# rvaser/rala

Measured on AMD Instinct MI355X. Metric: overlaps/sec (pile build + transitive reduction), higher is better.
Workload: dtype u16/u32 (+f64 compares)

## Files before the change

rala_amd/csrc/context.h:

```cpp
#pragma once

#include <hip/hip_runtime.h>
#include <stdint.h>

#include <algorithm>

#include <memory>
#include <string>
#include <vector>

#include "geom.h"
#include "host_pool.h"
#include "kernels.h"
#include "rala_hip.h"

namespace rala_hip {

struct HostOvl {
    uint32_t src;
    uint32_t a, b;
    Coords c;
    uint8_t strand;
    uint8_t dead;
    uint8_t type;
// ... 141 lines not shown
    uint32_t n_compute_units = 256;
    hipStream_t stream = nullptr;
    hipStream_t side = nullptr;
    hipStream_t aux = nullptr;
    bool use_side_stream = true;
    std::string err;
    hipEvent_t ev[12] = {};
    hipStream_t copy = nullptr;
    hipEvent_t ev_up[4] = {};
    bool upload_pending = false, upload_queued = false;
    const uint32_t* up_src[7] = {};
    const uint8_t* up_strand = nullptr;

    int64_t pool_per_read_x1000 = 1000;
    int64_t max_lds_read_len = 22000;
    int64_t debug_pile_stop_after = 99;
    int64_t host_threads = 0;
    std::unique_ptr<rala_hip::HostPool> pool;
    bool use_run_kernel = true;
    bool debug_fail_construct = false;
    uint32_t debug_pile_variant = 0;
    uint32_t debug_dedupe_list_cap = 0;
    uint32_t debug_fp_lds_limit = 0xFFFFFFFFu;
    uint32_t debug_fp_give_up = 0;
    int64_t debug_chunk_fail = -1;
    uint32_t debug_part_shift = 0;
    uint32_t debug_count_window = 0;
    bool use_bound_records = true;
    bool use_round_batches = true;
    rala_hip::DevBuf<uint32_t> d_round_log;

    uint64_t n_reads = 0;
    uint32_t max_read_len = 0;
    uint32_t n_class[rala_hip::kPileClasses] = {};
    rala_hip::DevBuf<uint32_t> d_class_order;
    rala_hip::DevBuf<uint32_t> d_seg_base;
    rala_hip::DevBuf<uint32_t> d_dense;
    std::vector<uint32_t> h_read_len;
    std::vector<uint64_t> h_pile_off;
    uint64_t pile_elems = 0;
    rala_hip::DevBuf<uint32_t> d_read_len;
    rala_hip::DevBuf<uint64_t> d_pile_off;
    rala_hip::DevBuf<uint16_t> d_pile;
    rala_hip::DevBuf<uint32_t> d_order, d_overflow;
    rala_hip::DevBuf<uint32_t> d_big_list[2], d_big_space;
    int64_t debug_big_caps = 0;
// ... 159 lines not shown
```

rala_amd/csrc/kernels.h:

```cpp
#pragma once

#include <hip/hip_runtime.h>
#include <stdint.h>

namespace rala_hip {

constexpr uint32_t kPadL = 848;

enum : uint32_t {
    kErrRegionCapacity = 1u,
    kErrPoolCapacity = 2u,
    kErrRawCapacity = 4u,
};

struct Interval {
    uint32_t first, second;
    uint32_t aux;
};

struct PileArgs {
    const uint32_t* read_len;
    const uint64_t* pile_off;
    uint16_t* pile;
    const uint32_t* ev_off;
// ... 214 lines not shown
void launch_sens_filter(const TailList& L, const uint32_t* begin, const uint32_t* end, const uint32_t* n_rep,
                        const uint32_t* rep_slot, const Interval* rep_pool, hipStream_t s);
void launch_finalize_states(const TailList& L, const uint8_t* alive, hipStream_t s);
void launch_list_targets(const uint32_t* off, uint32_t n, uint32_t* list, uint32_t* count, hipStream_t s);
void launch_list_members(const uint32_t* alive_reads, const uint8_t* touched, uint32_t n_alive, uint32_t world, uint32_t rank,
                         uint32_t* list, uint32_t* count, hipStream_t s);
struct SensSplitArgs {
    const uint32_t* read_len;
    const uint32_t* ev_off;
    const uint32_t* ev_cnt;
    uint32_t ev_stride;
    uint32_t ev_shift;
    const uint32_t* sens_off;
    const uint32_t* begin;
    const uint32_t* end;
    uint32_t* out[5];
    uint32_t* counts;
};
void launch_sens_split(const uint32_t* list, uint32_t bound, const uint32_t* n_dev, const SensSplitArgs& args, hipStream_t s);
void launch_status_clear(uint32_t* status, uint32_t bits, uint32_t* zero, hipStream_t s);
void launch_scatter_component_medians(const uint32_t* alive_reads, const uint8_t* touched, const uint16_t* cmed, uint32_t n_alive,
                                      uint16_t* out, hipStream_t s);
void launch_break_hills(const TailReads& R, uint32_t n_reads, hipStream_t s);
void launch_break_pits(const TailReads& R, const uint32_t* alive_reads, const uint8_t* touched, const uint16_t* comp_median,
                       uint32_t n_alive, hipStream_t s, const uint32_t* gate = nullptr);
void launch_retrim(const TailList& L, const TailReads& R, uint32_t promote, uint32_t round, uint32_t* dropped,
                   hipStream_t s, const uint32_t* gate = nullptr);
void launch_cc_edges(const TailList& L, const uint32_t* rank, uint32_t* edges, uint8_t* touched, uint32_t* label, uint32_t n_labels,
                     hipStream_t s);
void launch_refresh_types(const TailList& L, const TailReads& R, hipStream_t s);
hipError_t launch_tail_contain(const TailList& L, const TailReads& R, uint8_t* alive, uint32_t* const lists[6], uint32_t* zeroed21, uint32_t* const work[4],
                               uint32_t* base2, uint8_t* mark2, uint32_t* map, uint32_t* pack, uint32_t n_reads, uint32_t lds_limit, uint32_t debug_give_up, hipStream_t s);
void launch_count_zero_u8(const uint8_t* x, uint32_t n, uint32_t* out, hipStream_t s);
void launch_tail_init(const TailList& L, uint32_t n0, const TailReads& R, uint32_t* n_pits0, uint32_t n_reads, uint32_t* base2,
                      uint8_t* mark2, uint32_t* map, uint32_t* zero22, hipStream_t s);
struct ScanSpace;
bool launch_rank_pass(const uint8_t* alive, uint32_t* rank, uint32_t* alive_reads, uint32_t n_reads, ScanSpace& space, hipStream_t s);
bool launch_node_pass(const uint8_t* alive, uint32_t* node_rank, uint32_t* node_read, uint32_t* n_final, uint32_t n_reads,
                      ScanSpace& space, hipStream_t s);
bool launch_segment_pass(const TailList& L, const TailReads& R, uint32_t want_state, uint32_t want_round, uint32_t* base,
                         uint32_t* next, uint32_t* kept_item, const uint32_t* node_rank, uint32_t* e_src, uint32_t* e_dst,
                         uint32_t* e_len, ScanSpace& space, hipStream_t s);
bool launch_offsets_pass(const uint32_t* in, uint32_t* out, uint32_t* copy, uint32_t n, ScanSpace& space, hipStream_t s);
bool launch_pair_offsets_pass(const uint32_t* in0, const uint32_t* in1, uint32_t* out0, uint32_t* out1, uint32_t* totals, uint32_t n,
                              ScanSpace& space, hipStream_t s);

struct FixedPointList {
    const uint32_t *key, *target, *keeper;
    const uint32_t* count;
    uint32_t lds_limit = 0xFFFFFFFFu;
    uint32_t debug_give_up = 0;
};
size_t fixed_point_pack_words();
hipError_t launch_fixed_point_finish(const FixedPointList& list, uint32_t* base, uint32_t* map, uint32_t* pack, uint32_t* const work[4],
                                     uint32_t* sync8, uint32_t* error, uint32_t* rounds_out, hipStream_t s);
// ... 97 lines not shown
void launch_gzip_resolve(uint16_t* sym, const uint64_t* text_off, uint32_t n_true, uint64_t text_n, uint8_t* text, uint32_t* seg_crc,
                         uint32_t* flags, hipStream_t s);
uint32_t gzip_segment_bytes();
uint32_t gzip_crc_of_segments(const uint32_t* seg_crc, uint64_t text_n);

size_t scan_workspace_bytes(uint64_t n);
void launch_exclusive_scan(const uint32_t* in, uint32_t* out, uint64_t n, void* workspace, hipStream_t s);

void launch_tr_mark(const uint32_t* row_ptr, const uint32_t* adj_edge, const uint32_t* edge_src,
                    const uint32_t* edge_dst, const uint32_t* edge_len, uint32_t n_nodes, uint32_t first_edge,
                    uint32_t last_edge, uint8_t* marks, hipStream_t s);
void launch_tr_degree(const uint32_t* src, const uint32_t* dst, uint32_t n_nodes, uint32_t n_edges, uint32_t* deg,
                      uint32_t* bad, hipStream_t s);
void launch_tr_fill(const uint32_t* src, const uint32_t* dst, uint32_t n_nodes, uint32_t n_edges, uint32_t* cursor, uint32_t* adj,
                    hipStream_t s);
void launch_cc_init(uint32_t* label, uint32_t n, hipStream_t s);
void launch_cc_hook(const uint32_t* edges, uint32_t n_edges, uint32_t sample, uint32_t* label, uint32_t* changed,
                    hipStream_t s);
void launch_cc_compress(uint32_t* label, uint32_t n, hipStream_t s);
void launch_cc_compress_count(uint32_t* label, uint32_t n, const uint8_t* touched, uint32_t* size, hipStream_t s);
size_t component_median_workspace(uint32_t n);
void component_median_clear(void* tmp, uint32_t n, FillList& fills);
uint32_t* component_median_sizes(void* tmp, uint32_t n);
hipError_t launch_component_medians(const uint32_t* label, const uint8_t* touched, const uint32_t* alive_reads,
                                    const uint16_t* median, uint32_t n_alive, void* tmp, uint16_t* cmed, hipStream_t s);
void launch_tr_count(uint8_t* marks, uint32_t n_edges, uint32_t* n_pairs, hipStream_t s);

void launch_layout_step(uint32_t n, const double* x, const double* y, double* x_out, double* y_out,
                        const uint32_t* adj_off, const uint32_t* adj, double k, double t, hipStream_t s);

}
```

rala_amd/csrc/median_kernels.hip:

```cpp
#include <hip/hip_runtime.h>

#include "device_utils.h"
#include "kernels.h"
#include "scan_pass.h"

namespace rala_hip {

namespace {

constexpr int kBlock = 256;
constexpr int kSelectBlock = 1024;

struct MedianSpace {
    uint32_t *size, *cursor, *start;
    uint16_t *vals, *root;
    ScanSpace scan;
    size_t zero_bytes;
};

inline size_t align16(size_t b) { return (b + 15) & ~(size_t)15; }
inline MedianSpace median_space(void* tmp, uint32_t n) {
    MedianSpace m;
    unsigned char* p = (unsigned char*)tmp;
    m.size = (uint32_t*)p; p += align16((size_t)n * 4);
// ... 124 lines not shown
        if (tid == 0) root_median[r] = (uint16_t)(high << 8 | s_pick[0]);
    }
}

__global__ __launch_bounds__(kBlock) void median_spread_kernel(const uint32_t* __restrict__ label, const uint8_t* __restrict__ touched,
                                                               const uint16_t* __restrict__ root_median, uint32_t n,
                                                               uint16_t* __restrict__ cmed) {
    const uint32_t q = blockIdx.x * kBlock + threadIdx.x;
    if (q < n && touched[q]) cmed[q] = root_median[label[q]];
}

}

size_t component_median_workspace(uint32_t n) {
    return 2 * align16((size_t)n * 4) + ((size_t)scan_tiles_for(n) + 1) * 8 + 16 + align16((size_t)(n + 2) * 4) +
           2 * align16((size_t)n * 2) + 256;
}

void component_median_clear(void* tmp, uint32_t n, FillList& fills) {
    if (n) fills.add(tmp, 0, median_space(tmp, n).zero_bytes);
}

uint32_t* component_median_sizes(void* tmp, uint32_t n) { return median_space(tmp, n).size; }

hipError_t launch_component_medians(const uint32_t* label, const uint8_t* touched, const uint32_t* alive_reads,
                                    const uint16_t* median, uint32_t n_alive, void* tmp, uint16_t* cmed, hipStream_t s) {
    if (n_alive == 0) return hipSuccess;
    MedianSpace m = median_space(tmp, n_alive);
    if (!launch_offsets_pass(m.size, m.start, nullptr, n_alive, m.scan, s)) return hipErrorOutOfMemory;
    const dim3 grid((n_alive + kBlock - 1) / kBlock);
    hipLaunchKernelGGL(median_fill_kernel, grid, dim3(kBlock), 0, s, label, touched, alive_reads, median, n_alive,
                       (const uint32_t*)m.start, m.cursor, m.vals);
    hipLaunchKernelGGL(median_select_kernel, dim3((n_alive + kSelectBlock - 1) / kSelectBlock), dim3(kSelectBlock), 0, s, label,
                       (const uint32_t*)m.size, (const uint32_t*)m.start, (const uint16_t*)m.vals, n_alive, m.root);
    hipLaunchKernelGGL(median_spread_kernel, grid, dim3(kBlock), 0, s, label, touched, (const uint16_t*)m.root, n_alive, cmed);
    return hipGetLastError();
}

}
```

rala_amd/csrc/pipeline.hip:

```cpp
#include <hip/hip_runtime.h>
#include <stdio.h>
#include <stdlib.h>
#include <string.h>

#include <algorithm>
#include <chrono>
#include <numeric>

#include "context.h"
#include "scan_pass.h"
#include "stages.h"

using namespace rala_hip;


hipError_t rala_hip::d2h_small(rala_hip_ctx* ctx, void* dst, const void* src, size_t bytes, hipStream_t s) {
    if (ctx->p_stage.ensure(256) != hipSuccess || ctx->stage_used + bytes > 256 * sizeof(uint32_t) ||
        ctx->stage_pending.size() >= 16) {
        return hipMemcpyAsync(dst, src, bytes, hipMemcpyDeviceToHost, s);
    }
    char* at = (char*)ctx->p_stage.p + ctx->stage_used;
    const hipError_t e = hipMemcpyAsync(at, src, bytes, hipMemcpyDeviceToHost, s);
    if (e != hipSuccess) return e;
    ctx->stage_pending.push_back({dst, ctx->stage_used, bytes});
    ctx->stage_used += (bytes + 7) & ~(size_t)7;
    return hipSuccess;
}

hipError_t rala_hip::stream_sync(rala_hip_ctx* ctx, hipStream_t s) {
    const hipError_t e = hipStreamSynchronize(s);
    if (e == hipSuccess) {
        for (const auto& c : ctx->stage_pending) memcpy(c.dst, (const char*)ctx->p_stage.p + c.offset, c.bytes);
    }
    ctx->stage_pending.clear();
    ctx->stage_used = 0;
    return e;
}

namespace {

#define HIPCHECK(call)                                                                       \
    do {                                                                                     \
        hipError_t e_ = (call);                                                              \
        if (e_ != hipSuccess) {                                                              \
            ctx->err = std::string(#call) + ": " + hipGetErrorString(e_);                    \
            ctx->stage_pending.clear();                                                      \
            ctx->stage_used = 0;                                                             \
            return e_ == hipErrorOutOfMemory ? RALA_HIP_ENOMEM : RALA_HIP_EDEVICE;           \
        }                                                                                    \
    } while (0)

int fail(rala_hip_ctx* ctx, int code, const char* msg) {
    ctx->err = msg;
    ctx->stage_pending.clear();
    ctx->stage_used = 0;
    return code;
}

ReadState read_state(rala_hip_ctx* ctx) {
    ReadState rs;
    rs.begin = ctx->d_begin.p; rs.end = ctx->d_end.p; rs.alive = ctx->d_alive.p;
    rs.n_pits = ctx->d_n_pits.p; rs.n_hills = ctx->d_n_hills.p; rs.iv_slot = ctx->d_iv_slot.p;
// ... 674 lines not shown
            if (x + kHillFuzz > h[i].first && h[i].aux) return false;
        }
    }
    return true;
}

int materialize_host(rala_hip_ctx* ctx);
int download_repeat_hills(rala_hip_ctx* ctx) {
    if (!ctx->rep_host_stale) return RALA_HIP_OK;
    const uint64_t n = ctx->n_reads;
    HIPCHECK(hipSetDevice(ctx->device));
    ctx->h_n_rep.resize(n); ctx->h_rep_slot.resize(n);
    HIPCHECK(hipMemcpy(ctx->h_n_rep.data(), ctx->d_n_rep.p, n * 4, hipMemcpyDeviceToHost));
    HIPCHECK(hipMemcpy(ctx->h_rep_slot.data(), ctx->d_rep_slot.p, n * 4, hipMemcpyDeviceToHost));
    ctx->h_rep_pool.resize(ctx->n_rep_hills);
    if (ctx->n_rep_hills) {
        HIPCHECK(hipMemcpy(ctx->h_rep_pool.data(), ctx->d_rep_pool.p, (size_t)ctx->n_rep_hills * sizeof(Interval), hipMemcpyDeviceToHost));
    }
    ctx->rep_host_stale = false;
    return RALA_HIP_OK;
}
void build_graph(rala_hip_ctx* ctx);
TailList tail_list(rala_hip_ctx* ctx);
int tail_components(rala_hip_ctx* ctx, const TailList& L, uint32_t n_alive, bool touched_cleared = false);
int gpu_tail_part_b(rala_hip_ctx* ctx);

int preprocess_repeats(rala_hip_ctx* cs, rala_hip_ctx* cl, Comm* comm, const rala_hip_overlaps* sens, uint64_t n_sens,
                       bool device_lists) {
    rala_hip_ctx* ctx = cs;
    const bool sharded = comm != nullptr;
    const uint32_t P = sharded ? comm->world() : 1u, me = sharded ? comm->rank() : 0u;
    const uint64_t n = cs->n_reads;
    const uint64_t nl = cl->n_reads;
    const uint64_t nl_pad = ((n + P - 1) / P + 15) / 16 * 16;
    hipStream_t s = cs->stream;
    hipStream_t sl = cl->stream;
    Trace trc;
    auto comm_fail = [&](const char* what) {
        cs->err = std::string(what) + ": " + comm->error();
        cs->stage_pending.clear();
        cs->stage_used = 0;
        return RALA_HIP_EDEVICE;
    };
    if (n_sens >= 0x7FFFFFF0ull / 2) return fail(ctx, RALA_HIP_EINVAL, "too many sensitive overlaps");
    OvlSoA so;
    {
        const uint32_t* src[7] = {nullptr, nullptr, nullptr, nullptr, nullptr, nullptr, nullptr};
// ... 435 lines not shown
    return L;
}

TailReads tail_reads(rala_hip_ctx* ctx) {
    TailReads R;
    R.begin = ctx->d_begin.p; R.end = ctx->d_end.p; R.alive = ctx->d_alive.p; R.dirty = ctx->d_dirty.p;
    R.n_pits = ctx->d_n_pits.p; R.n_hills = ctx->d_n_hills.p; R.n_pits0 = ctx->d_n_pits0.p;
    R.iv_slot = ctx->d_iv_slot.p; R.pool = ctx->d_pool.p;
    return R;
}

int scan_space(rala_hip_ctx* ctx, uint32_t scans, uint64_t items, ScanSpace& sp, FillList* fills) {
    const size_t words = (size_t)scans * (scan_tiles_for(items) + 2) + 2;
    HIPCHECK(ctx->d_scan_state.ensure(words));
    sp.state = ctx->d_scan_state.p;
    sp.words = words - 2;
    sp.used = 0;
    sp.ticket = (uint32_t*)(ctx->d_scan_state.p + words - 2);
    if (fills) fills->add(ctx->d_scan_state.p, 0, words * 8);
    else HIPCHECK(hipMemsetAsync(ctx->d_scan_state.p, 0, words * 8, ctx->stream));
    return RALA_HIP_OK;
}

int tail_components(rala_hip_ctx* ctx, const TailList& L, uint32_t n_alive, bool touched_cleared) {
    hipStream_t s = ctx->stream;
    const uint32_t M = L.n;
    if (!touched_cleared) {
        FillList fills;
        fills.add(ctx->d_touched.p, 0, n_alive);
        component_median_clear(ctx->d_med_tmp.p, n_alive, fills);
        HIPCHECK(fills.launch(s));
    }
    launch_cc_edges(L, ctx->d_rank.p, ctx->d_cc_edges.p, ctx->d_touched.p, ctx->d_cc_label.p, n_alive, s);
    for (int k = 0; k < 2; ++k) {
        launch_cc_hook(ctx->d_cc_edges.p, M, 1, ctx->d_cc_label.p, ctx->d_cc_flags.p + 7, s);
        launch_cc_compress(ctx->d_cc_label.p, n_alive, s);
    }
    launch_cc_hook(ctx->d_cc_edges.p, M, 0, ctx->d_cc_label.p, ctx->d_cc_flags.p + 7, s);
    launch_cc_compress_count(ctx->d_cc_label.p, n_alive, ctx->d_touched.p, component_median_sizes(ctx->d_med_tmp.p, n_alive), s);
    HIPCHECK(launch_component_medians(ctx->d_cc_label.p, ctx->d_touched.p, ctx->d_alive_reads.p, ctx->d_median.p, n_alive,
                                      ctx->d_med_tmp.p, ctx->d_cmed.p, s));
    return RALA_HIP_OK;
}

int gpu_tail_part_a(rala_hip_ctx* ctx) {
    hipStream_t s = ctx->stream;
    Trace trc;
    auto mark = [&](const char* what, size_t k = 0) {
        if (trc.on) { (void)stream_sync(ctx, s); trc(what, k); }
    };
    const uint32_t n_reads = (uint32_t)ctx->n_reads;
    const uint32_t M = ctx->t_n0 + ctx->t_n1;
    const uint32_t n_alive = ctx->t_n_alive;
    const size_t big = (size_t)std::max<uint64_t>(n_reads, M) + 2;
    HIPCHECK(ctx->d_t_state.ensure(M)); HIPCHECK(ctx->d_t_round.ensure(M));
    HIPCHECK(ctx->d_dirty.ensure(n_reads)); HIPCHECK(ctx->d_n_pits0.ensure(n_reads));
    HIPCHECK(ctx->d_rank.ensure(n_reads)); HIPCHECK(ctx->d_alive_reads.ensure(n_reads));
    HIPCHECK(ctx->d_kept_item.ensure(M));
    HIPCHECK(ctx->d_node_rank.ensure(n_reads + 2)); HIPCHECK(ctx->d_t_death[0].ensure(n_reads));
    HIPCHECK(ctx->d_t_death[1].ensure(n_reads));
    HIPCHECK(ctx->d_touched.ensure(n_alive)); HIPCHECK(ctx->d_cmed.ensure(n_alive));
    HIPCHECK(ctx->d_cc_edges.ensure(2 * (size_t)M)); HIPCHECK(ctx->d_cc_label.ensure(n_alive));
    ctx->t_med_tmp = component_median_workspace(n_alive);
    HIPCHECK(ctx->d_med_tmp.ensure(ctx->t_med_tmp));
// ... 10 lines not shown
        HIPCHECK(fills.launch(s));
    }
    HIPCHECK(ctx->d_counts.ensure(48));
    for (int k = 0; k < 2; ++k) HIPCHECK(ctx->d_t_work[k].ensure(n_reads));
    HIPCHECK(ctx->d_t_fin.ensure(2 * (size_t)n_reads));
    HIPCHECK(ctx->d_t_mark.ensure(2 * (size_t)n_reads));
    for (int k = 0; k < 3; ++k) { HIPCHECK(ctx->d_kill[k].ensure((size_t)M + 1)); HIPCHECK(ctx->d_kill2[k].ensure((size_t)M + 1)); }
    HIPCHECK(ctx->d_fp_map.ensure(n_reads));
    HIPCHECK(ctx->d_fp_pack.ensure(fixed_point_pack_words()));
    launch_tail_init(L, ctx->t_n0, R, ctx->d_n_pits0.p, n_reads, ctx->d_t_fin.p, ctx->d_t_mark.p, ctx->d_fp_map.p, ctx->d_counts.p + 9, s);
    if (!launch_rank_pass(ctx->d_alive.p, ctx->d_rank.p, ctx->d_alive_reads.p, n_reads, sp, s)) return fail(ctx, RALA_HIP_EDEVICE, "scan space");
    mark("tail: ranks", n_alive);

    HIPCHECK(ctx->d_counts.ensure(48));
    uint32_t* dropped = ctx->d_counts.p + 4;
    launch_break_hills(R, n_reads, s);
    if (ctx->lists_pending) {
        HIPCHECK(hipStreamWaitEvent(s, ctx->ev[3], 0));
        ctx->lists_pending = false;
    }
    launch_retrim(L, R, 0, 0, dropped, s);
    mark("tail: hills + retrim", M);

    uint32_t rounds = 0;
    for (;;) {
        const uint32_t batch = rounds == 0 ? 2u : 1u;
        for (uint32_t k = 0; k < batch; ++k) {
            if (rounds + k >= 255) return fail(ctx, RALA_HIP_EDEVICE, "chimera loop did not settle");
            const uint32_t* gate = k ? dropped + k - 1 : nullptr;
            FillList fills;
            fills.add(ctx->d_dirty.p, 0, n_reads);
            fills.add(ctx->d_touched.p, 0, n_alive);
            component_median_clear(ctx->d_med_tmp.p, n_alive, fills);
            if (k == 0) fills.add(dropped, 0, 2 * 4);
            HIPCHECK(fills.launch(s));
            const int rcc = tail_components(ctx, L, n_alive, true);
            if (rcc != RALA_HIP_OK) return rcc;
            launch_break_pits(R, ctx->d_alive_reads.p, ctx->d_touched.p, ctx->d_cmed.p, n_alive, s, gate);
            launch_retrim(L, R, 1, rounds + k, dropped + k, s, gate);
        }
        uint32_t d[2] = {0, 0};
        HIPCHECK(d2h_small(ctx, d, dropped, sizeof(d), s));
        HIPCHECK(stream_sync(ctx, s));
        mark("tail: pits + retrim", d[0] + d[1]);
        if (!d[0]) { rounds += 1; break; }
        rounds += batch;
        if (!d[batch - 1]) break;
    }
    ctx->t_rounds = rounds;
    if ((uint64_t)M * ((uint64_t)rounds + 2ull) >= 0xFFFFFFF0ull) {
        return fail(ctx, RALA_HIP_ETOOLARGE, "too many surviving overlaps for 32-bit list positions");
    }

    {
        uint32_t* const work[4] = {ctx->d_t_death[0].p, ctx->d_t_death[1].p, ctx->d_t_work[0].p, ctx->d_t_work[1].p};
        uint32_t* const lists[6] = {ctx->d_kill[0].p, ctx->d_kill[1].p, ctx->d_kill[2].p, ctx->d_kill2[0].p, ctx->d_kill2[1].p,
                                    ctx->d_kill2[2].p};
        HIPCHECK(launch_tail_contain(L, R, ctx->d_alive.p, lists, ctx->d_counts.p + 9, work, ctx->d_t_fin.p, ctx->d_t_mark.p, ctx->d_fp_map.p,
                                     ctx->d_fp_pack.p, n_reads, ctx->debug_fp_lds_limit, ctx->debug_fp_give_up, s));
    }
    mark("tail: containment scans", M);
    return RALA_HIP_OK;
}

int gpu_tail_part_b(rala_hip_ctx* ctx) {
    hipStream_t s = ctx->stream;
    Trace trc;
    auto mark = [&](const char* what, size_t k = 0) {
        if (trc.on) { (void)stream_sync(ctx, s); trc(what, k); }
    };
    const uint32_t n_reads = (uint32_t)ctx->n_reads;
    const uint32_t M = ctx->t_n0 + ctx->t_n1;
    const TailList L = tail_list(ctx);
    const TailReads R = tail_reads(ctx);
    const uint32_t n_seg = ctx->t_rounds + 1;
    HIPCHECK(ctx->d_seg_base.ensure(2 * (size_t)n_seg + 4));
    HIPCHECK(ctx->d_node_read.ensure(2 * (size_t)ctx->t_n_alive + 2));
    for (int k = 0; k < 3; ++k) HIPCHECK(ctx->d_e[k].ensure(2 * (size_t)M + 2));
    HIPCHECK(ctx->d_counts.ensure(48));
    ScanSpace sp;
    {
        FillList fills;
        const int rc = scan_space(ctx, n_seg + 1, std::max<uint64_t>(n_reads, M), sp, &fills);
// ... 596 lines not shown

int rala_hip_set_option(rala_hip_ctx* ctx, const char* key, int64_t value) {
    if (!ctx || !key) return RALA_HIP_EINVAL;
    if (!strcmp(key, "interval_pool_per_read_x1000")) { ctx->pool_per_read_x1000 = value; return RALA_HIP_OK; }
    if (!strcmp(key, "debug_big_caps")) { ctx->debug_big_caps = value; return RALA_HIP_OK; }
    if (!strcmp(key, "debug_force_big")) { ctx->debug_force_big = value != 0; return RALA_HIP_OK; }
    if (!strcmp(key, "max_lds_read_len")) { ctx->max_lds_read_len = value; return RALA_HIP_OK; }
    if (!strcmp(key, "debug_pile_stop_after")) { ctx->debug_pile_stop_after = value; return RALA_HIP_OK; }
    if (!strcmp(key, "use_run_kernel")) { ctx->use_run_kernel = value != 0; return RALA_HIP_OK; }
    if (!strcmp(key, "use_round_batches")) { ctx->use_round_batches = value != 0; return RALA_HIP_OK; }
    if (!strcmp(key, "use_bound_records")) { ctx->use_bound_records = value != 0; return RALA_HIP_OK; }
    if (!strcmp(key, "use_fused_emit")) { ctx->use_fused_emit = value != 0; return RALA_HIP_OK; }
    if (!strcmp(key, "ingest_window_bytes")) { ctx->ingest_window_bytes = std::max<int64_t>(0, value); return RALA_HIP_OK; }
    if (!strcmp(key, "gzip_on_device")) { ctx->gzip_on_device = value != 0; return RALA_HIP_OK; }
    if (!strcmp(key, "gzip_chunk_bytes")) { ctx->gzip_chunk_bytes = value > 0 ? value : 64 << 10; return RALA_HIP_OK; }
    if (!strcmp(key, "debug_gzip_false_sync")) { ctx->debug_gzip_false_sync = (uint32_t)std::max<int64_t>(0, value); return RALA_HIP_OK; }
    if (!strcmp(key, "pile_chunk_mb")) { ctx->pile_chunk_mb = (uint32_t)std::max<int64_t>(0, std::min<int64_t>(value, 1 << 20)); return RALA_HIP_OK; }
    if (!strcmp(key, "debug_ev_events")) { ctx->debug_ev_events = value != 0; return RALA_HIP_OK; }
    if (!strcmp(key, "debug_count_window")) { ctx->debug_count_window = (uint32_t)std::max<int64_t>(0, value); return RALA_HIP_OK; }
    if (!strcmp(key, "debug_part_shift")) { ctx->debug_part_shift = (uint32_t)std::max<int64_t>(0, value); return RALA_HIP_OK; }
    if (!strcmp(key, "debug_pile_variant")) { ctx->debug_pile_variant = (uint32_t)std::max<int64_t>(0, value); return RALA_HIP_OK; }
    if (!strcmp(key, "debug_dedupe_list_cap")) { ctx->debug_dedupe_list_cap = (uint32_t)std::max<int64_t>(0, value); return RALA_HIP_OK; }
    if (!strcmp(key, "debug_fp_lds_limit")) { ctx->debug_fp_lds_limit = (uint32_t)std::max<int64_t>(0, value); return RALA_HIP_OK; }
    if (!strcmp(key, "debug_fp_give_up")) { ctx->debug_fp_give_up = value == 2 ? 2u : value != 0 ? 1u : 0u; return RALA_HIP_OK; }
    if (!strcmp(key, "debug_chunk_fail")) { ctx->debug_chunk_fail = value; return RALA_HIP_OK; }
    if (!strcmp(key, "debug_fail_construct")) { ctx->debug_fail_construct = value != 0; return RALA_HIP_OK; }
    if (!strcmp(key, "use_gpu_tail")) { ctx->use_gpu_tail = value != 0; return RALA_HIP_OK; }
    if (!strcmp(key, "use_fixed_buckets")) { ctx->use_fixed_buckets = value != 0; return RALA_HIP_OK; }
    if (!strcmp(key, "use_partitioned_buckets")) { ctx->use_partitioned_buckets = value != 0; return RALA_HIP_OK; }
    if (!strcmp(key, "use_side_stream")) { ctx->use_side_stream = value != 0; return RALA_HIP_OK; }
    if (!strcmp(key, "sensitive_in_device_memory")) { ctx->sens_in_device = value != 0; return RALA_HIP_OK; }
    if (!strcmp(key, "host_threads")) {
        ctx->host_threads = value;
        ctx->pool.reset(new HostPool((unsigned)std::max<int64_t>(1, std::min<int64_t>(value, 256))));
        return RALA_HIP_OK;
    }
    return fail(ctx, RALA_HIP_EINVAL, "unknown option");
}

void* rala_hip_stream(rala_hip_ctx* ctx) { return ctx ? (void*)ctx->stream : nullptr; }

int rala_hip_set_reads(rala_hip_ctx* ctx, const uint32_t* read_len, uint64_t n_reads) {
    if (!ctx || (!read_len && n_reads)) return RALA_HIP_EINVAL;
    if (n_reads >= 0x7FFFFFFFull) return fail(ctx, RALA_HIP_EINVAL, "too many reads");
    HIPCHECK(hipSetDevice(ctx->device));
    HIPCHECK(hipStreamSynchronize(ctx->side));
// ... 1081 lines not shown
```

rala_amd/csrc/tail_kernels.hip:

```cpp
#include <hip/hip_runtime.h>

#include <algorithm>

#include "device_utils.h"
#include "geom.h"
#include "kernels.h"
#include "scan_pass.h"

namespace rala_hip {

namespace {

constexpr int kBlock = 256;
constexpr uint32_t kInf = 0xFFFFFFFFu;

inline dim3 grid_for(uint64_t n) { return dim3((unsigned)((n + kBlock - 1) / kBlock)); }

__device__ __forceinline__ bool dev_shrink(const TailReads& R, uint32_t r, uint32_t b, uint32_t e) {
    if (b > e || e - b < kMinRegion) { R.dirty[r] = 1; return false; }
    if (R.begin[r] != b || R.end[r] != e) R.dirty[r] = 1;
    R.begin[r] = b;
    R.end[r] = e;
    return true;
}

__global__ __launch_bounds__(kBlock) void break_hills_kernel(TailReads R, uint32_t n_reads) {
    const uint32_t r = blockIdx.x * kBlock + threadIdx.x;
    if (r >= n_reads || !R.alive[r] || R.n_hills[r] == 0) return;
    const Interval* hills = R.pool + R.iv_slot[r] + R.n_pits0[r];
    const Piece keep = longest_piece(R.begin[r], R.end[r], R.n_hills[r],
                                     [&](uint32_t i, uint32_t& f, uint32_t& s) { f = hills[i].first; s = hills[i].second; },
                                     [&](uint32_t i) { return hills[i].aux <= 3; });
    if (!dev_shrink(R, r, keep.begin, keep.end)) R.alive[r] = 0;
    R.n_hills[r] = 0;
}

__global__ __launch_bounds__(kBlock) void break_pits_kernel(TailReads R, const uint32_t* __restrict__ alive_reads,
                                                            const uint8_t* __restrict__ touched,
                                                            const uint16_t* __restrict__ comp_median, uint32_t n_alive,
                                                            const uint32_t* gate) {
    if (gate && *gate == 0) return;
    const uint32_t q = blockIdx.x * kBlock + threadIdx.x;
    if (q >= n_alive || !touched[q]) return;
    const uint32_t r = alive_reads[q];
    if (!R.alive[r] || R.n_pits[r] == 0) return;
    Interval* pits = R.pool + R.iv_slot[r];
    const double med = (double)comp_median[q];
    uint32_t w = 0;
    const Piece keep = longest_piece(R.begin[r], R.end[r], R.n_pits[r],
                                     [&](uint32_t k, uint32_t& f, uint32_t& s) { f = pits[k].first; s = pits[k].second; },
                                     [&](uint32_t k) {
                                         if ((double)pits[k].aux * 1.84 <= med) return true;
                                         pits[w++] = pits[k];
                                         return false;
                                     });
    R.n_pits[r] = w;
    if (!dev_shrink(R, r, keep.begin, keep.end)) R.alive[r] = 0;
}

__device__ __forceinline__ Coords item_coords(const TailList& L, uint32_t k) {
    Coords c;
    c.a_begin = L.a_begin[k]; c.a_end = L.a_end[k]; c.b_begin = L.b_begin[k]; c.b_end = L.b_end[k];
    c.length = L.length[k];
    return c;
}

__global__ __launch_bounds__(kBlock) void retrim_kernel(TailList L, TailReads R, uint32_t promote, uint32_t round,
                                                        uint32_t* dropped, const uint32_t* gate) {
    if (gate && *gate == 0) return;
    const uint32_t k = blockIdx.x * kBlock + threadIdx.x;
// ... 182 lines not shown
                                                                    const uint32_t* __restrict__ base0,
                                                                    const uint32_t* __restrict__ base1) {
    const uint32_t k = blockIdx.x * kBlock + threadIdx.x;
    if (k >= L.n) return;
    const uint8_t st = L.state[k];
    if (st == 0) return;
    const uint8_t t = L.type[k];
    bool drop = t == kTypeA || t == kTypeB;
    if (st == 2 && !drop) {
        const uint32_t a = L.a[k], b = L.b[k];
        drop = gone_before_second_scan(alive, base0, a) || gone_before_second_scan(alive, base0, b) || base1[a] < k || base1[b] < k;
    }
    if (drop) L.state[k] = 0;
}

__global__ __launch_bounds__(kBlock) void tail_contain_kill_kernel(TailKillers K, uint32_t n_items, uint8_t* alive) {
    const uint32_t n0 = K.count[0], n1 = K.count[1];
    for (uint32_t i = blockIdx.x * kBlock + threadIdx.x; i < n0 + n1; i += gridDim.x * kBlock) {
        const uint32_t target = K.target[i < n0 ? i : n_items - 1u - (i - n0)];
        if (K.base[0][target] != kInf || K.base[1][target] != kInf) alive[target] = 0;
    }
}

__global__ __launch_bounds__(kBlock) void tail_init_kernel(uint8_t* state, uint8_t* round, uint32_t n0, uint32_t m,
                                                           uint8_t* dirty, uint32_t* n_pits0, const uint32_t* n_pits,
                                                           uint32_t n_reads, uint32_t* base2, uint8_t* mark2, uint32_t* map, uint32_t* zero22) {
    const uint32_t k = blockIdx.x * kBlock + threadIdx.x;
    if (k < 22) zero22[k] = 0;
    if (k < n_reads) {
        base2[k] = kInf; base2[n_reads + k] = kInf; map[k] = kInf;
        mark2[k] = 0; mark2[n_reads + k] = 0;
    }
    if (k < m) {
        state[k] = k < n0 ? 1 : 2;
        round[k] = 0;
    }
    if (k < n_reads) {
        dirty[k] = 0;
        n_pits0[k] = n_pits[k];
    }
}

struct RankPass {
    const uint8_t* alive;
    uint32_t* rank;
    uint32_t* alive_reads;
// ... 72 lines not shown
    __device__ void total(uint64_t sum) const { out[n] = (uint32_t)sum; }
};

struct PairOffsetsPass {
    const uint32_t *in0, *in1;
    uint32_t *out0, *out1, *totals;
    uint32_t n;
    __device__ uint64_t value(uint32_t i) const { return (uint64_t)in0[i] | (uint64_t)in1[i] << 31; }
    __device__ void place(uint32_t i, uint64_t, uint64_t before) const {
        out0[i] = (uint32_t)(before & 0x7FFFFFFFull);
        out1[i] = (uint32_t)(before >> 31);
    }
    __device__ void total(uint64_t sum) const {
        out0[n] = totals[0] = (uint32_t)(sum & 0x7FFFFFFFull);
        out1[n] = totals[1] = (uint32_t)(sum >> 31);
    }
};

}

void launch_break_hills(const TailReads& R, uint32_t n_reads, hipStream_t s) {
    if (n_reads) hipLaunchKernelGGL(break_hills_kernel, grid_for(n_reads), dim3(kBlock), 0, s, R, n_reads);
}
void launch_break_pits(const TailReads& R, const uint32_t* alive_reads, const uint8_t* touched, const uint16_t* comp_median,
                       uint32_t n_alive, hipStream_t s, const uint32_t* gate) {
    if (n_alive) {
        hipLaunchKernelGGL(break_pits_kernel, grid_for(n_alive), dim3(kBlock), 0, s, R, alive_reads, touched, comp_median,
                           n_alive, gate);
    }
}
void launch_retrim(const TailList& L, const TailReads& R, uint32_t promote, uint32_t round, uint32_t* dropped,
                   hipStream_t s, const uint32_t* gate) {
    if (L.n) hipLaunchKernelGGL(retrim_kernel, grid_for(L.n), dim3(kBlock), 0, s, L, R, promote, round, dropped, gate);
}
void launch_cc_edges(const TailList& L, const uint32_t* rank, uint32_t* edges, uint8_t* touched, uint32_t* label, uint32_t n_labels,
                     hipStream_t s) {
    const uint32_t n = std::max<uint32_t>(L.n, n_labels);
    if (n) hipLaunchKernelGGL(cc_edges_kernel, grid_for(n), dim3(kBlock), 0, s, L, rank, edges, touched, label, n_labels);
}
void launch_refresh_types(const TailList& L, const TailReads& R, hipStream_t s) {
    if (L.n) hipLaunchKernelGGL(refresh_types_kernel, grid_for(L.n), dim3(kBlock), 0, s, L, R);
}
hipError_t launch_tail_contain(const TailList& L, const TailReads& R, uint8_t* alive, uint32_t* const lists[6], uint32_t* zeroed21, uint32_t* const work[4],
                               uint32_t* base2, uint8_t* mark2, uint32_t* map, uint32_t* pack, uint32_t n_reads, uint32_t lds_limit, uint32_t debug_give_up, hipStream_t s) {
    if (!L.n) return hipSuccess;
    TailKillers K;
    K.key = lists[0]; K.target = lists[1]; K.keeper = lists[2];
    K.c_key = lists[3]; K.c_target = lists[4]; K.c_keeper = lists[5];
    K.error = zeroed21; K.count = zeroed21 + 1;
    K.mark[0] = mark2; K.mark[1] = mark2 + n_reads;
    K.base[0] = base2; K.base[1] = base2 + n_reads;
    const uint32_t per_block = kCollectPer * kContainBlock;
    hipLaunchKernelGGL(tail_contain_collect_kernel, dim3((L.n + per_block - 1) / per_block), dim3(kContainBlock), 0, s, L, R,
                       (const uint8_t*)alive, K);
    for (int c = 0; c < 2; ++c) {
        if (c == 0) hipLaunchKernelGGL(tail_contain_reduce_kernel<0>, dim3(128), dim3(kBlock), 0, s, K, L.n, (const uint8_t*)alive);
        else hipLaunchKernelGGL(tail_contain_reduce_kernel<1>, dim3(128), dim3(kBlock), 0, s, K, L.n, (const uint8_t*)alive);
        const FixedPointList conditional = {K.c_key, K.c_target, K.c_keeper, K.count + 2 + c, lds_limit, debug_give_up};
        const hipError_t e = launch_fixed_point_finish(conditional, K.base[c], map, pack, work, zeroed21 + 5 + 8 * c, K.error, nullptr, s);
        if (e != hipSuccess) return e;
    }
    hipLaunchKernelGGL(tail_contain_apply_kernel, grid_for(L.n), dim3(kBlock), 0, s, L, (const uint8_t*)alive,
                       (const uint32_t*)K.base[0], (const uint32_t*)K.base[1]);
    hipLaunchKernelGGL(tail_contain_kill_kernel, dim3(128), dim3(kBlock), 0, s, K, L.n, alive);
    return hipGetLastError();
}
void launch_tail_init(const TailList& L, uint32_t n0, const TailReads& R, uint32_t* n_pits0, uint32_t n_reads, uint32_t* base2,
                      uint8_t* mark2, uint32_t* map, uint32_t* zero22, hipStream_t s) {
    const uint32_t n = std::max<uint32_t>(std::max<uint32_t>(L.n, n_reads), 22u);
    hipLaunchKernelGGL(tail_init_kernel, grid_for(n), dim3(kBlock), 0, s, L.state, L.round, n0, L.n, R.dirty, n_pits0, R.n_pits, n_reads,
                       base2, mark2, map, zero22);
}
bool launch_rank_pass(const uint8_t* alive, uint32_t* rank, uint32_t* alive_reads, uint32_t n_reads, ScanSpace& space, hipStream_t s) {
    return launch_scan_pass(n_reads, RankPass{alive, rank, alive_reads}, space, s);
}
bool launch_node_pass(const uint8_t* alive, uint32_t* node_rank, uint32_t* node_read, uint32_t* n_final, uint32_t n_reads,
                      ScanSpace& space, hipStream_t s) {
    return launch_scan_pass(n_reads, NodePass{alive, node_rank, node_read, n_final}, space, s);
}
bool launch_segment_pass(const TailList& L, const TailReads& R, uint32_t want_state, uint32_t want_round, uint32_t* base,
                         uint32_t* next, uint32_t* kept_item, const uint32_t* node_rank, uint32_t* e_src, uint32_t* e_dst,
                         uint32_t* e_len, ScanSpace& space, hipStream_t s) {
    SegmentPass f;
    f.L = L; f.R = R; f.want_state = want_state; f.want_round = want_round; f.base = base; f.kept_item = kept_item;
    f.node_rank = node_rank; f.e_src = e_src; f.e_dst = e_dst; f.e_len = e_len; f.next = next;
    return launch_scan_pass(L.n, f, space, s);
}
bool launch_pair_offsets_pass(const uint32_t* in0, const uint32_t* in1, uint32_t* out0, uint32_t* out1, uint32_t* totals, uint32_t n,
// ... 20 lines not shown
```

Measured before the change: 7.269 billion.

## Speculatively run containment scans during first pit-round host sync; fuse median spread

After the first pit/retrim batch, the containment scan kernels are enqueued speculatively before the host waits on the dropped counts, so GPU work overlaps the host sync. If more rounds follow, a reset kernel clears the scan state and the scans run again at the end. Separately, the component-median spread kernel is folded into break_pits, which reads the root median through the label directly. The trade-off is wasted scan work plus an extra reset launch whenever the speculation misses.

```diff
diff --git a/rala_amd/csrc/context.h b/rala_amd/csrc/context.h
--- a/rala_amd/csrc/context.h
+++ b/rala_amd/csrc/context.h
@@ -187,6 +187,7 @@
     uint32_t debug_pile_variant = 0;
     uint32_t debug_dedupe_list_cap = 0;
     uint32_t debug_fp_lds_limit = 0xFFFFFFFFu;
+    bool debug_tail_rescan = false;
     uint32_t debug_fp_give_up = 0;
     int64_t debug_chunk_fail = -1;
     uint32_t debug_part_shift = 0;
diff --git a/rala_amd/csrc/kernels.h b/rala_amd/csrc/kernels.h
--- a/rala_amd/csrc/kernels.h
+++ b/rala_amd/csrc/kernels.h
@@ -260,15 +260,19 @@
 void launch_scatter_component_medians(const uint32_t* alive_reads, const uint8_t* touched, const uint16_t* cmed, uint32_t n_alive,
                                       uint16_t* out, hipStream_t s);
 void launch_break_hills(const TailReads& R, uint32_t n_reads, hipStream_t s);
-void launch_break_pits(const TailReads& R, const uint32_t* alive_reads, const uint8_t* touched, const uint16_t* comp_median,
-                       uint32_t n_alive, hipStream_t s, const uint32_t* gate = nullptr);
+void launch_break_pits(const TailReads& R, const uint32_t* alive_reads, const uint8_t* touched, uint16_t* comp_median,
+                       uint32_t n_alive, hipStream_t s, const uint32_t* gate = nullptr, const uint32_t* label = nullptr,
+                       const uint16_t* root_median = nullptr);
 void launch_retrim(const TailList& L, const TailReads& R, uint32_t promote, uint32_t round, uint32_t* dropped,
                    hipStream_t s, const uint32_t* gate = nullptr);
 void launch_cc_edges(const TailList& L, const uint32_t* rank, uint32_t* edges, uint8_t* touched, uint32_t* label, uint32_t n_labels,
                      hipStream_t s);
 void launch_refresh_types(const TailList& L, const TailReads& R, hipStream_t s);
 hipError_t launch_tail_contain(const TailList& L, const TailReads& R, uint8_t* alive, uint32_t* const lists[6], uint32_t* zeroed21, uint32_t* const work[4],
-                               uint32_t* base2, uint8_t* mark2, uint32_t* map, uint32_t* pack, uint32_t n_reads, uint32_t lds_limit, uint32_t debug_give_up, hipStream_t s);
+                               uint32_t* base2, uint8_t* mark2, uint32_t* map, uint32_t* pack, uint32_t n_reads, uint32_t lds_limit, uint32_t debug_give_up, hipStream_t s,
+                               uint32_t parts = 3u);
+constexpr uint32_t kTailContainScans = 1u, kTailContainApply = 2u;
+void launch_tail_contain_reset(uint32_t n_reads, uint32_t* base2, uint8_t* mark2, uint32_t* map, uint32_t* zero22, hipStream_t s);
 void launch_count_zero_u8(const uint8_t* x, uint32_t n, uint32_t* out, hipStream_t s);
 void launch_tail_init(const TailList& L, uint32_t n0, const TailReads& R, uint32_t* n_pits0, uint32_t n_reads, uint32_t* base2,
                       uint8_t* mark2, uint32_t* map, uint32_t* zero22, hipStream_t s);
@@ -412,8 +416,10 @@
 size_t component_median_workspace(uint32_t n);
 void component_median_clear(void* tmp, uint32_t n, FillList& fills);
 uint32_t* component_median_sizes(void* tmp, uint32_t n);
+const uint16_t* component_median_roots(void* tmp, uint32_t n);
 hipError_t launch_component_medians(const uint32_t* label, const uint8_t* touched, const uint32_t* alive_reads,
-                                    const uint16_t* median, uint32_t n_alive, void* tmp, uint16_t* cmed, hipStream_t s);
+                                    const uint16_t* median, uint32_t n_alive, void* tmp, uint16_t* cmed, hipStream_t s,
+                                    bool spread = true);
 void launch_tr_count(uint8_t* marks, uint32_t n_edges, uint32_t* n_pairs, hipStream_t s);
 
 void launch_layout_step(uint32_t n, const double* x, const double* y, double* x_out, double* y_out,
diff --git a/rala_amd/csrc/median_kernels.hip b/rala_amd/csrc/median_kernels.hip
--- a/rala_amd/csrc/median_kernels.hip
+++ b/rala_amd/csrc/median_kernels.hip
@@ -170,9 +170,10 @@
 }
 
 uint32_t* component_median_sizes(void* tmp, uint32_t n) { return median_space(tmp, n).size; }
+const uint16_t* component_median_roots(void* tmp, uint32_t n) { return median_space(tmp, n).root; }
 
 hipError_t launch_component_medians(const uint32_t* label, const uint8_t* touched, const uint32_t* alive_reads,
-                                    const uint16_t* median, uint32_t n_alive, void* tmp, uint16_t* cmed, hipStream_t s) {
+                                    const uint16_t* median, uint32_t n_alive, void* tmp, uint16_t* cmed, hipStream_t s, bool spread) {
     if (n_alive == 0) return hipSuccess;
     MedianSpace m = median_space(tmp, n_alive);
     if (!launch_offsets_pass(m.size, m.start, nullptr, n_alive, m.scan, s)) return hipErrorOutOfMemory;
@@ -181,7 +182,7 @@
                        (const uint32_t*)m.start, m.cursor, m.vals);
     hipLaunchKernelGGL(median_select_kernel, dim3((n_alive + kSelectBlock - 1) / kSelectBlock), dim3(kSelectBlock), 0, s, label,
                        (const uint32_t*)m.size, (const uint32_t*)m.start, (const uint16_t*)m.vals, n_alive, m.root);
-    hipLaunchKernelGGL(median_spread_kernel, grid, dim3(kBlock), 0, s, label, touched, (const uint16_t*)m.root, n_alive, cmed);
+    if (spread) hipLaunchKernelGGL(median_spread_kernel, grid, dim3(kBlock), 0, s, label, touched, (const uint16_t*)m.root, n_alive, cmed);
     return hipGetLastError();
 }
 
diff --git a/rala_amd/csrc/pipeline.hip b/rala_amd/csrc/pipeline.hip
--- a/rala_amd/csrc/pipeline.hip
+++ b/rala_amd/csrc/pipeline.hip
@@ -38,6 +38,16 @@
 }
 
 namespace {
+
+hipError_t event_sync(rala_hip_ctx* ctx, hipEvent_t ev) {
+    const hipError_t e = hipEventSynchronize(ev);
+    if (e == hipSuccess) {
+        for (const auto& c : ctx->stage_pending) memcpy(c.dst, (const char*)ctx->p_stage.p + c.offset, c.bytes);
+    }
+    ctx->stage_pending.clear();
+    ctx->stage_used = 0;
+    return e;
+}
 
 #define HIPCHECK(call)                                                                       \
     do {                                                                                     \
@@ -758,7 +768,7 @@
 }
 void build_graph(rala_hip_ctx* ctx);
 TailList tail_list(rala_hip_ctx* ctx);
-int tail_components(rala_hip_ctx* ctx, const TailList& L, uint32_t n_alive, bool touched_cleared = false);
+int tail_components(rala_hip_ctx* ctx, const TailList& L, uint32_t n_alive, bool touched_cleared = false, bool spread_later = false);
 int gpu_tail_part_b(rala_hip_ctx* ctx);
 
 int preprocess_repeats(rala_hip_ctx* cs, rala_hip_ctx* cl, Comm* comm, const rala_hip_overlaps* sens, uint64_t n_sens,
@@ -1240,7 +1250,7 @@
     return RALA_HIP_OK;
 }
 
-int tail_components(rala_hip_ctx* ctx, const TailList& L, uint32_t n_alive, bool touched_cleared) {
+int tail_components(rala_hip_ctx* ctx, const TailList& L, uint32_t n_alive, bool touched_cleared, bool spread_later) {
     hipStream_t s = ctx->stream;
     const uint32_t M = L.n;
     if (!touched_cleared) {
@@ -1257,7 +1267,7 @@
     launch_cc_hook(ctx->d_cc_edges.p, M, 0, ctx->d_cc_label.p, ctx->d_cc_flags.p + 7, s);
     launch_cc_compress_count(ctx->d_cc_label.p, n_alive, ctx->d_touched.p, component_median_sizes(ctx->d_med_tmp.p, n_alive), s);
     HIPCHECK(launch_component_medians(ctx->d_cc_label.p, ctx->d_touched.p, ctx->d_alive_reads.p, ctx->d_median.p, n_alive,
-                                      ctx->d_med_tmp.p, ctx->d_cmed.p, s));
+                                      ctx->d_med_tmp.p, ctx->d_cmed.p, s, !spread_later));
     return RALA_HIP_OK;
 }
 
@@ -1314,6 +1324,14 @@
     launch_retrim(L, R, 0, 0, dropped, s);
     mark("tail: hills + retrim", M);
 
+    uint32_t* const contain_work[4] = {ctx->d_t_death[0].p, ctx->d_t_death[1].p, ctx->d_t_work[0].p, ctx->d_t_work[1].p};
+    uint32_t* const contain_lists[6] = {ctx->d_kill[0].p, ctx->d_kill[1].p, ctx->d_kill[2].p, ctx->d_kill2[0].p, ctx->d_kill2[1].p,
+                                        ctx->d_kill2[2].p};
+    auto contain = [&](uint32_t parts) {
+        return launch_tail_contain(L, R, ctx->d_alive.p, contain_lists, ctx->d_counts.p + 9, contain_work, ctx->d_t_fin.p, ctx->d_t_mark.p,
+                                   ctx->d_fp_map.p, ctx->d_fp_pack.p, n_reads, ctx->debug_fp_lds_limit, ctx->debug_fp_give_up, s, parts);
+    };
+    bool scans_ahead = false;
     uint32_t rounds = 0;
     for (;;) {
         const uint32_t batch = rounds == 0 ? 2u : 1u;
@@ -1326,31 +1344,38 @@
             component_median_clear(ctx->d_med_tmp.p, n_alive, fills);
             if (k == 0) fills.add(dropped, 0, 2 * 4);
             HIPCHECK(fills.launch(s));
-            const int rcc = tail_components(ctx, L, n_alive, true);
+            const int rcc = tail_components(ctx, L, n_alive, true, true);
             if (rcc != RALA_HIP_OK) return rcc;
-            launch_break_pits(R, ctx->d_alive_reads.p, ctx->d_touched.p, ctx->d_cmed.p, n_alive, s, gate);
+            launch_break_pits(R, ctx->d_alive_reads.p, ctx->d_touched.p, ctx->d_cmed.p, n_alive, s, gate, ctx->d_cc_label.p,
+                              component_median_roots(ctx->d_med_tmp.p, n_alive));
             launch_retrim(L, R, 1, rounds + k, dropped + k, s, gate);
         }
         uint32_t d[2] = {0, 0};
         HIPCHECK(d2h_small(ctx, d, dropped, sizeof(d), s));
-        HIPCHECK(stream_sync(ctx, s));
+        if (rounds == 0 && (uint64_t)M * 4ull < 0xFFFFFFF0ull) {
+            HIPCHECK(hipEventRecord(ctx->ev[10], s));
+            HIPCHECK(contain(kTailContainScans));
+            scans_ahead = true;
+            HIPCHECK(event_sync(ctx, ctx->ev[10]));
+        } else {
+            HIPCHECK(stream_sync(ctx, s));
+        }
         mark("tail: pits + retrim", d[0] + d[1]);
-        if (!d[0]) { rounds += 1; break; }
-        rounds += batch;
-        if (!d[batch - 1]) break;
+        const bool done = !d[0] || !d[batch - 1];
+        rounds += d[0] ? batch : 1u;
+        if (done && !ctx->debug_tail_rescan) break;
+        if (scans_ahead) {
+            launch_tail_contain_reset(n_reads, ctx->d_t_fin.p, ctx->d_t_mark.p, ctx->d_fp_map.p, ctx->d_counts.p + 9, s);
+            scans_ahead = false;
+        }
+        if (done) break;
     }
     ctx->t_rounds = rounds;
     if ((uint64_t)M * ((uint64_t)rounds + 2ull) >= 0xFFFFFFF0ull) {
         return fail(ctx, RALA_HIP_ETOOLARGE, "too many surviving overlaps for 32-bit list positions");
     }
 
-    {
-        uint32_t* const work[4] = {ctx->d_t_death[0].p, ctx->d_t_death[1].p, ctx->d_t_work[0].p, ctx->d_t_work[1].p};
-        uint32_t* const lists[6] = {ctx->d_kill[0].p, ctx->d_kill[1].p, ctx->d_kill[2].p, ctx->d_kill2[0].p, ctx->d_kill2[1].p,
-                                    ctx->d_kill2[2].p};
-        HIPCHECK(launch_tail_contain(L, R, ctx->d_alive.p, lists, ctx->d_counts.p + 9, work, ctx->d_t_fin.p, ctx->d_t_mark.p, ctx->d_fp_map.p,
-                                     ctx->d_fp_pack.p, n_reads, ctx->debug_fp_lds_limit, ctx->debug_fp_give_up, s));
-    }
+    HIPCHECK(contain(scans_ahead ? kTailContainApply : kTailContainScans | kTailContainApply));
     mark("tail: containment scans", M);
     return RALA_HIP_OK;
 }
@@ -1993,6 +2018,7 @@
     if (!strcmp(key, "debug_pile_variant")) { ctx->debug_pile_variant = (uint32_t)std::max<int64_t>(0, value); return RALA_HIP_OK; }
     if (!strcmp(key, "debug_dedupe_list_cap")) { ctx->debug_dedupe_list_cap = (uint32_t)std::max<int64_t>(0, value); return RALA_HIP_OK; }
     if (!strcmp(key, "debug_fp_lds_limit")) { ctx->debug_fp_lds_limit = (uint32_t)std::max<int64_t>(0, value); return RALA_HIP_OK; }
+    if (!strcmp(key, "debug_tail_rescan")) { ctx->debug_tail_rescan = value != 0; return RALA_HIP_OK; }
     if (!strcmp(key, "debug_fp_give_up")) { ctx->debug_fp_give_up = value == 2 ? 2u : value != 0 ? 1u : 0u; return RALA_HIP_OK; }
     if (!strcmp(key, "debug_chunk_fail")) { ctx->debug_chunk_fail = value; return RALA_HIP_OK; }
     if (!strcmp(key, "debug_fail_construct")) { ctx->debug_fail_construct = value != 0; return RALA_HIP_OK; }
diff --git a/rala_amd/csrc/tail_kernels.hip b/rala_amd/csrc/tail_kernels.hip
--- a/rala_amd/csrc/tail_kernels.hip
+++ b/rala_amd/csrc/tail_kernels.hip
@@ -37,15 +37,19 @@
 
 __global__ __launch_bounds__(kBlock) void break_pits_kernel(TailReads R, const uint32_t* __restrict__ alive_reads,
                                                             const uint8_t* __restrict__ touched,
-                                                            const uint16_t* __restrict__ comp_median, uint32_t n_alive,
-                                                            const uint32_t* gate) {
-    if (gate && *gate == 0) return;
+                                                            uint16_t* comp_median, uint32_t n_alive,
+                                                            const uint32_t* gate, const uint32_t* __restrict__ label,
+                                                            const uint16_t* __restrict__ root_median) {
     const uint32_t q = blockIdx.x * kBlock + threadIdx.x;
     if (q >= n_alive || !touched[q]) return;
+    uint16_t cm;
+    if (root_median) { cm = root_median[label[q]]; comp_median[q] = cm; }
+    else cm = comp_median[q];
+    if (gate && *gate == 0) return;
     const uint32_t r = alive_reads[q];
     if (!R.alive[r] || R.n_pits[r] == 0) return;
     Interval* pits = R.pool + R.iv_slot[r];
-    const double med = (double)comp_median[q];
+    const double med = (double)cm;
     uint32_t w = 0;
     const Piece keep = longest_piece(R.begin[r], R.end[r], R.n_pits[r],
                                      [&](uint32_t k, uint32_t& f, uint32_t& s) { f = pits[k].first; s = pits[k].second; },
@@ -274,6 +278,16 @@
     }
 }
 
+__global__ __launch_bounds__(kBlock) void tail_contain_reset_kernel(uint32_t n_reads, uint32_t* base2, uint8_t* mark2, uint32_t* map,
+                                                                    uint32_t* zero22) {
+    const uint32_t k = blockIdx.x * kBlock + threadIdx.x;
+    if (k < 22) zero22[k] = 0;
+    if (k < n_reads) {
+        base2[k] = kInf; base2[n_reads + k] = kInf; map[k] = kInf;
+        mark2[k] = 0; mark2[n_reads + k] = 0;
+    }
+}
+
 __global__ __launch_bounds__(kBlock) void tail_init_kernel(uint8_t* state, uint8_t* round, uint32_t n0, uint32_t m,
                                                            uint8_t* dirty, uint32_t* n_pits0, const uint32_t* n_pits,
                                                            uint32_t n_reads, uint32_t* base2, uint8_t* mark2, uint32_t* map, uint32_t* zero22) {
@@ -392,11 +406,11 @@
 void launch_break_hills(const TailReads& R, uint32_t n_reads, hipStream_t s) {
     if (n_reads) hipLaunchKernelGGL(break_hills_kernel, grid_for(n_reads), dim3(kBlock), 0, s, R, n_reads);
 }
-void launch_break_pits(const TailReads& R, const uint32_t* alive_reads, const uint8_t* touched, const uint16_t* comp_median,
-                       uint32_t n_alive, hipStream_t s, const uint32_t* gate) {
+void launch_break_pits(const TailReads& R, const uint32_t* alive_reads, const uint8_t* touched, uint16_t* comp_median,
+                       uint32_t n_alive, hipStream_t s, const uint32_t* gate, const uint32_t* label, const uint16_t* root_median) {
     if (n_alive) {
         hipLaunchKernelGGL(break_pits_kernel, grid_for(n_alive), dim3(kBlock), 0, s, R, alive_reads, touched, comp_median,
-                           n_alive, gate);
+                           n_alive, gate, label, root_median);
     }
 }
 void launch_retrim(const TailList& L, const TailReads& R, uint32_t promote, uint32_t round, uint32_t* dropped,
@@ -412,7 +426,8 @@
     if (L.n) hipLaunchKernelGGL(refresh_types_kernel, grid_for(L.n), dim3(kBlock), 0, s, L, R);
 }
 hipError_t launch_tail_contain(const TailList& L, const TailReads& R, uint8_t* alive, uint32_t* const lists[6], uint32_t* zeroed21, uint32_t* const work[4],
-                               uint32_t* base2, uint8_t* mark2, uint32_t* map, uint32_t* pack, uint32_t n_reads, uint32_t lds_limit, uint32_t debug_give_up, hipStream_t s) {
+                               uint32_t* base2, uint8_t* mark2, uint32_t* map, uint32_t* pack, uint32_t n_reads, uint32_t lds_limit, uint32_t debug_give_up, hipStream_t s,
+                               uint32_t parts) {
     if (!L.n) return hipSuccess;
     TailKillers K;
     K.key = lists[0]; K.target = lists[1]; K.keeper = lists[2];
@@ -421,19 +436,25 @@
     K.mark[0] = mark2; K.mark[1] = mark2 + n_reads;
     K.base[0] = base2; K.base[1] = base2 + n_reads;
     const uint32_t per_block = kCollectPer * kContainBlock;
-    hipLaunchKernelGGL(tail_contain_collect_kernel, dim3((L.n + per_block - 1) / per_block), dim3(kContainBlock), 0, s, L, R,
+    if (parts & kTailContainScans) hipLaunchKernelGGL(tail_contain_collect_kernel, dim3((L.n + per_block - 1) / per_block), dim3(kContainBlock), 0, s, L, R,
                        (const uint8_t*)alive, K);
-    for (int c = 0; c < 2; ++c) {
+    for (int c = 0; c < 2 && (parts & kTailContainScans); ++c) {
         if (c == 0) hipLaunchKernelGGL(tail_contain_reduce_kernel<0>, dim3(128), dim3(kBlock), 0, s, K, L.n, (const uint8_t*)alive);
         else hipLaunchKernelGGL(tail_contain_reduce_kernel<1>, dim3(128), dim3(kBlock), 0, s, K, L.n, (const uint8_t*)alive);
         const FixedPointList conditional = {K.c_key, K.c_target, K.c_keeper, K.count + 2 + c, lds_limit, debug_give_up};
         const hipError_t e = launch_fixed_point_finish(conditional, K.base[c], map, pack, work, zeroed21 + 5 + 8 * c, K.error, nullptr, s);
         if (e != hipSuccess) return e;
     }
-    hipLaunchKernelGGL(tail_contain_apply_kernel, grid_for(L.n), dim3(kBlock), 0, s, L, (const uint8_t*)alive,
-                       (const uint32_t*)K.base[0], (const uint32_t*)K.base[1]);
-    hipLaunchKernelGGL(tail_contain_kill_kernel, dim3(128), dim3(kBlock), 0, s, K, L.n, alive);
+    if (parts & kTailContainApply) {
+        hipLaunchKernelGGL(tail_contain_apply_kernel, grid_for(L.n), dim3(kBlock), 0, s, L, (const uint8_t*)alive,
+                           (const uint32_t*)K.base[0], (const uint32_t*)K.base[1]);
+        hipLaunchKernelGGL(tail_contain_kill_kernel, dim3(128), dim3(kBlock), 0, s, K, L.n, alive);
+    }
     return hipGetLastError();
+}
+void launch_tail_contain_reset(uint32_t n_reads, uint32_t* base2, uint8_t* mark2, uint32_t* map, uint32_t* zero22, hipStream_t s) {
+    hipLaunchKernelGGL(tail_contain_reset_kernel, grid_for(std::max<uint32_t>(n_reads, 22u)), dim3(kBlock), 0, s, n_reads, base2, mark2,
+                       map, zero22);
 }
 void launch_tail_init(const TailList& L, uint32_t n0, const TailReads& R, uint32_t* n_pits0, uint32_t n_reads, uint32_t* base2,
                       uint8_t* mark2, uint32_t* map, uint32_t* zero22, hipStream_t s) {
```

New measurement: 7.263 billion. No clear change (-0.1%).
